# alshai/pfbwt-f

Measured on AMD Instinct MI355X. Metric: Gbases/s end-to-end BWT+SA build; bit-exact .bwt/.sa vs reference, higher is better.
Workload: dtype u8 text / u32 indices / u64 hash; 1 GPU; S-32G; L=32000000, H=1000, seed=1000, w=10, p=100, flags=-r, uint_t=64, n=32000010000, r=83625322, input=text resident in HBM, outputs (.bwt, .ssa, .esa) left in HBM, per_rank=single GPU

## Files before the change

### pfbwt-f_amd/csrc/common.h

```cpp
#pragma once
#include <hip/hip_runtime.h>
#include <cstdint>
#include <cstdio>
#include <cstdlib>
#include <cstring>
#include <chrono>
#include <string>
#include <vector>
#include "../../include/pfbwt_hip.h"
#include "devmem.h"
#include "../../include/pfbwt_hip_dev.h"

namespace pfp {

typedef uint32_t idx_t;

constexpr int BLOCK = 256;
constexpr int WAVE = 64;

constexpr uint8_t Dollar = 2, EndOfWord = 1, EndOfDict = 0;

enum KernelId {
    K_TRIGGER_SCAN, K_PHRASE_ENDS, K_PHRASE_HASH, K_PHRASE_HASH_LONG, K_DEDUP_HEADS, K_DEDUP_LONG,
    K_DICT_BUILD, K_RADIX_HIST, K_RADIX_SCATTER, K_SCAN_REDUCE, K_SCAN_SPINE, K_SCAN_APPLY,
// ... 31 lines not shown
        return base + hi;
    }
    void *reserve_lo(size_t bytes)
    {
        size_t a = (lo + 255) & ~(size_t)255;
        if (a + bytes > hi) { failed = true; want += bytes; return nullptr; }
        lo = a + bytes;
        return base + a;
    }
    bool commit_range(const void *p, size_t bytes) { const size_t o = (size_t)((const char *)p - base); return vm.commit(o, o + bytes); }
    size_t offset_of(const void *p) const { return (size_t)((const char *)p - base); }
    size_t mark_hi() const { return hi; }
    void release_hi(size_t m) { hi = m; }
    size_t mark_lo() const { return lo; }
    void release_lo(size_t m) { lo = m; }
};

struct Tunables {
    int verbose = 0;
    int seg_grid = 768;
    int seg_stage = 1;
    int sort_k = 0;
    int sort_no_table = 0;
    uint32_t class_sort_maxrange = 0;
    int dedup_table_log2 = 0;
    int no_trigger_table = 0;
    uint64_t emit_chunk_rows = 3ULL << 30;
    uint32_t fill_subs = 2;
    uint64_t sample_cap = ~0ULL;
    int no_runaware = 0;
    long big_group_members = -2;
    int force_wide_rows = 0;
    uint64_t ingest_block_bytes = 0;
    int expand_dma = 1;
    int ingest_readers = 0;
    uint32_t emit_group_rows = 4096;
    int dict_text_rounds = -1;
    int force_run_round = 0;
    int int_key_symbols = 3;
    int no_slot_records = 0;
    int group_reduce = 1;
    uint64_t fasta_chunk_bytes = 0;
    int parse_rec = -1;
    int parse_rec_p2 = 4;
    uint64_t parse_rec_min = 1u << 21;
    int parse_rec_depth = 1;
    uint32_t parse_rec_tile_rows = 0;
    int dict_rec = -1;
    int dict_rec_p2 = 16;
    int dedup_variant = -1;
    int64_t dedup_period = 0;
    int64_t dedup_chunk = 0;
    int dedup_packed = 1;
    int dedup_phases = 0;
    int parse_rec_table_log2 = 0;
    uint32_t doc_lds_max = 8192;
};

}

struct pfp_ctx {
    int w = 10; uint64_t p = 100; unsigned flags = 0; int device = 0;
    hipStream_t stream = nullptr;
    pfp::Arena arena;
    size_t arena_request = 0;
    uint64_t err_pos = 0; int err_ch = 0;
    pfp::VmRegion text;
    uint8_t *tb = nullptr; size_t tb_cap = 0; uint64_t n = 0; uint64_t text_hint = 0; uint64_t nseq = 0 ;
    struct RowViewPending { const uint8_t *src = nullptr; uint64_t count = 0, len = 0, stride = 0; } view;
    uint64_t left_ctx = 0;
    uint64_t tb_n = 0;
    int stage = 0;
    uint64_t m = 0, dwords = 0, dsize = 0;
    uint64_t *d_ye = nullptr;
    uint32_t *d_pid = nullptr;
    uint32_t *d_parse = nullptr;
    uint8_t *d_last = nullptr;
    uint8_t *d_dict = nullptr;
    uint32_t *d_ws = nullptr;
    uint32_t *d_wordid = nullptr;
    uint32_t *d_wrank = nullptr;
    uint32_t *d_occ = nullptr;
    uint8_t *d_sdict = nullptr;
    uint32_t *d_gsa = nullptr;
    uint8_t *d_sflag = nullptr;
    uint32_t *d_srank = nullptr;
    uint2 *d_grank = nullptr;
    bool gsa_valid = false;
    uint64_t nrows = 0;
    uint8_t *d_bwlast = nullptr; uint32_t *d_ilist = nullptr; uint64_t *d_bwsai = nullptr;
    uint8_t *d_bwl_il = nullptr;
    uint64_t nout = 0, runs = 0, esa_pairs = 0, easy = 0, hard = 0, slice_begin = 0, slice_rows = 0;
    uint8_t *d_bwt = nullptr; void *d_sa = nullptr; void *d_ssa = nullptr; void *d_esa = nullptr;
    bool have_sa = false, have_rssa = false;
    uint64_t *d_ma = nullptr; uint64_t ma_words = 0;
    size_t ma_lo_mark = (size_t)-1, ma_lo_end = 0;
    void *d_da = nullptr, *d_sda = nullptr, *d_eda = nullptr;
    size_t da_lo_mark = (size_t)-1, da_lo_end = 0;
    size_t lo_after_parse = 0, lo_after_pbwt = 0, emit_scratch_mark = 0;
    bool prof_on = false; uint64_t prof_mask = ~0ULL;
    pfp::ProfRec prof[pfp::K_COUNT_];
    struct PendingEv { hipEvent_t a, b; int id; double bytes; };
    std::vector<PendingEv> pending;
    std::vector<hipEvent_t> ev_pool;
    double stage_ms[3] = {0, 0, 0};
    int hip_err = 0;
    uint8_t *hstage[2] = {nullptr, nullptr}; hipEvent_t hstage_ev[2] = {nullptr, nullptr}; bool hstage_used[2] = {false, false};
    pfp::Tunables tun;
    struct FastaIngest {
        uint8_t *raw[2] = {nullptr, nullptr}; size_t rawcap = 0; bool used[2] = {false, false};
        hipStream_t copy = nullptr; bool copy_ready = false; hipEvent_t ev_copied[2] = {nullptr, nullptr}, ev_free[2] = {nullptr, nullptr};
        uint8_t *tiles = nullptr; size_t tiles_cap = 0;
        unsigned long long *d_tot = nullptr, *h_tot = nullptr;
        uint32_t state = 2; bool started = false; uint64_t records = 0;
        std::vector<uint64_t> rec_raw, rec_pos;
    } fa;
    uint8_t *h_bwt = nullptr; void *h_sa = nullptr;
    uint8_t *ing_buf[16] = {};
    uint64_t ing_next_off = 0;
    std::vector<std::string> doc_names; std::vector<uint64_t> doc_starts;
    uint64_t hash_seed = 0x9E3779B97F4A7C15ULL;
    uint32_t *d_trigtab = nullptr;
};

namespace pfp {

inline hipEvent_t ev_get(pfp_ctx *c)
{
    if (!c->ev_pool.empty()) { hipEvent_t e = c->ev_pool.back(); c->ev_pool.pop_back(); return e; }
    hipEvent_t e; (void)hipEventCreate(&e); return e;
}
inline void prof_collect(pfp_ctx *c)
{
    if (c->pending.empty()) return;
    (void)hipStreamSynchronize(c->stream);
    for (auto &pe : c->pending) {
        float ms = 0; (void)hipEventElapsedTime(&ms, pe.a, pe.b);
        c->prof[pe.id].launches++; c->prof[pe.id].ms += ms; c->prof[pe.id].bytes += pe.bytes;
        c->ev_pool.push_back(pe.a); c->ev_pool.push_back(pe.b);
    }
    c->pending.clear();
}
struct ProfScope {
    pfp_ctx *c; int id; double bytes; hipEvent_t a = nullptr; bool on = false;
    ProfScope(pfp_ctx *c_, int id_, double bytes_) : c(c_), id(id_), bytes(bytes_)
    {
        on = c->prof_on && ((c->prof_mask >> id) & 1ULL);
        if (on) { a = ev_get(c); (void)hipEventRecord(a, c->stream); }
    }
    ~ProfScope()
    {
        if (on) {
            hipEvent_t b = ev_get(c); (void)hipEventRecord(b, c->stream);
            c->pending.push_back({a, b, id, bytes});
            if (c->pending.size() > 4096) prof_collect(c);
        }
    }
};

#define PFP_LAUNCH(ctx, id, bytes, kernel, grid, ...)                                             \
    do {                                                                                          \
        pfp::ProfScope ps_((ctx), (id), (double)(bytes));                                         \
        if ((ctx)->tun.verbose >= 3) { fprintf(stderr, "[pfbwt_hip] launch %s grid %u\n", #kernel, (unsigned)(grid)); fflush(stderr); } \
        hipLaunchKernelGGL(kernel, dim3((unsigned)(grid)), dim3(pfp::BLOCK), 0, (ctx)->stream, __VA_ARGS__); \
        hipError_t le_ = hipGetLastError();             \
        if ((ctx)->tun.verbose >= 3 && le_ == hipSuccess) le_ = hipStreamSynchronize((ctx)->stream);    \
        if (le_ != hipSuccess) { (ctx)->hip_err = (int)le_; (ctx)->err_ch = (int)le_;                 \
            fprintf(stderr, "[pfbwt_hip] launch of %s failed: %s (%s:%d)\n", #kernel, hipGetErrorString(le_), __FILE__, __LINE__); \
            return PFP_E_HIP; }                                                                       \
    } while (0)

#define PFP_LAUNCH_B(ctx, id, bytes, kernel, grid, block, ...)                                    \
    do {                                                                                          \
        pfp::ProfScope ps_((ctx), (id), (double)(bytes));                                         \
// ... 34 lines not shown
```

### pfbwt-f_amd/csrc/parse.h

```cpp
#pragma once
#include "prims.h"

namespace pfp {

typedef uint64_t tpos_t;

__host__ __device__ __forceinline__ uint64_t wang_hash(uint64_t key)
{
    key = (~key) + (key << 21);
    key = key ^ (key >> 24);
    key = (key + (key << 3)) + (key << 8);
    key = key ^ (key >> 14);
    key = (key + (key << 2)) + (key << 4);
    key = key ^ (key >> 28);
    key = key + (key << 31);
    return key;
}

__device__ __forceinline__ uint32_t norm_base(uint32_t c, bool ntoa)
{
    if (c >= 'a' && c <= 'z') c -= 32;
    if (ntoa && !(c == 'A' || c == 'C' || c == 'G' || c == 'T')) c = 'A';
    return c;
}
// ... 15 lines not shown
{
    const uint64_t i = (uint64_t)blockIdx.x * BLOCK + threadIdx.x;
    if (i >= count * (uint64_t)w) return;
    const uint64_t row = i / (uint64_t)w, k = i - row * (uint64_t)w;
    dst[row * pitch + len + k] = 'A';
}

__device__ __forceinline__ uint32_t ntoa_code(uint32_t c)
{
    return (c == 'A' || c == 'N') ? 0u : (c == 'C') ? 1u : (c == 'G') ? 2u : (c == 'T' || c == '-') ? 3u : 5u;
}

__device__ __forceinline__ uint32_t lut8x4(uint32_t hi, uint32_t lo, uint32_t sel)
{
    return __builtin_amdgcn_perm(hi, lo, sel);
}
__device__ __forceinline__ uint32_t pack4(uint32_t x, bool ntoa, uint32_t *bad, uint32_t *out)
{
    const uint32_t h4 = (x >> 1) & 0x07070707u;
    const uint32_t exp4 = lut8x4(0x4E2D0000u, 0x47544341u, h4);
    const uint32_t L = (exp4 & 0x40404040u) >> 1;
    const uint32_t allowed = (x ^ exp4) & ~L;
    uint32_t nz = (((allowed & 0x7F7F7F7Fu) + 0x7F7F7F7Fu) | allowed) & 0x80808080u;
    uint32_t c4 = lut8x4(0x00030000u, 0x02030100u, h4);
    if (ntoa) {
        nz |= (h4 & 0x04040404u) << 5;
        const uint32_t m = (nz >> 7) * 0xFFu;
        *out = (exp4 & ~m) | (0x41414141u & m); c4 &= ~m; *bad = 0;
    } else {
        const uint32_t m = (nz >> 7) * 0xFFu;
        const uint32_t t = x & 0x7F7F7F7Fu;
        const uint32_t lower = (t + 0x1F1F1F1Fu) & ~(t + 0x05050505u) & ~x & 0x80808080u;
        *out = (exp4 & ~m) | ((x ^ (lower >> 2)) & m);
        c4 &= ~m;
        *bad = (((nz >> 7) * 0x01020408u) >> 24) & 0xFu;
    }
    return (c4 * 0x40100401u) >> 24;
}
__device__ __forceinline__ uint32_t pack16(const uint4 &q, bool ntoa, uint32_t *bad , uint4 *normed)
{
    const uint32_t wds[4] = {q.x, q.y, q.z, q.w};
    uint32_t out[4], pk = 0, badm = 0;
#pragma unroll
    for (int i = 0; i < 4; ++i) {
        uint32_t b4;
        pk = (pk << 8) | pack4(wds[i], ntoa, &b4, &out[i]);
        badm |= b4 << (4 * i);
    }
    *bad = badm;
    if (normed) *normed = make_uint4(out[0], out[1], out[2], out[3]);
    return pk;
}

struct DedupText { const uint32_t *Xp; const unsigned long long *Xc; uint64_t nwords; unsigned long long *stats ; };
__device__ __forceinline__ uint32_t codes_lsb_first(uint32_t x)
{
    x = ((x >> 2) & 0x33333333u) | ((x & 0x33333333u) << 2);
    x = ((x >> 4) & 0x0F0F0F0Fu) | ((x & 0x0F0F0F0Fu) << 4);
    return __builtin_bswap32(x);
}
__device__ __forceinline__ bool acgt16(const uint4 &v)
{
    const uint32_t wds[4] = {v.x, v.y, v.z, v.w};
    bool ok = true;
#pragma unroll
    for (int i = 0; i < 4; ++i) {
        const uint32_t h = (wds[i] >> 1) & 0x07070707u;
        ok = ok && wds[i] == lut8x4(0x4E2D0000u, 0x47544341u, h) && !(h & 0x04040404u);
    }
    return ok;
}
__device__ __forceinline__ uint32_t decode4(uint32_t b)
{
    uint32_t s = (b | (b << 12)) & 0x000F000Fu;
    s = (s | (s << 6)) & 0x03030303u;
    return lut8x4(0u, 0x54474341u, s);
}
__device__ __forceinline__ uint64_t decode8(uint32_t x16) { return ((uint64_t)decode4((x16 >> 8) & 0xFFu) << 32) | decode4(x16 & 0xFFu); }

struct DivTest { uint64_t dinv, limit; int k; };
inline DivTest make_divtest(uint64_t p)
{
    DivTest t; t.k = 0;
    uint64_t d = p;
    while (!(d & 1)) { d >>= 1; ++t.k; }
    uint64_t x = d;
    for (int i = 0; i < 5; ++i) x *= 2 - d * x;
    t.dinv = x; t.limit = ~0ULL / p;
    return t;
}
__host__ __device__ __forceinline__ bool divisible(uint64_t h, const DivTest &t)
{
    const uint64_t v = h * t.dinv;
    return (t.k ? ((v >> t.k) | (v << (64 - t.k))) : v) <= t.limit;
}
__global__ __launch_bounds__(BLOCK) void k_trigger_scan(uint8_t *X, uint64_t n, int w, DivTest p, uint64_t kmask, int ntoa,
                                                        uint16_t *mask16, uint64_t *blockcnt, unsigned long long *err_pos)
{
    __shared__ uint32_t pk[BLOCK + 2];
    __shared__ uint32_t red[4];
    const uint64_t t = (uint64_t)blockIdx.x * BLOCK + threadIdx.x;
    const uint64_t base = t * 16;
    uint4 q = make_uint4(0, 0, 0, 0), nq;
    uint32_t bad = 0;
    if (base < n) q = *reinterpret_cast<const uint4 *>(X + base);
    const uint32_t mine = pack16(q, ntoa != 0, &bad, &nq);
    if (base < n) {
        const uint32_t live = (n - base >= 16) ? 0xffffu : ((1u << (unsigned)(n - base)) - 1u);
        if (live != 0xffffu) {
            uint32_t a[4] = {q.x, q.y, q.z, q.w}, b[4] = {nq.x, nq.y, nq.z, nq.w};
            for (int i = 0; i < 16; ++i) if (!((live >> i) & 1)) { b[i >> 2] = (b[i >> 2] & ~(0xffu << (8 * (i & 3)))) | (a[i >> 2] & (0xffu << (8 * (i & 3)))); }
            nq = make_uint4(b[0], b[1], b[2], b[3]);
        }
        *reinterpret_cast<uint4 *>(X + base) = nq;
        bad &= live;
        if (bad) atomicMin(err_pos, (unsigned long long)(base + (uint64_t)(__ffs((int)bad) - 1)));
    }
    pk[threadIdx.x + 2] = mine;
    if (threadIdx.x < 2) {
        const uint64_t first = (uint64_t)blockIdx.x * BLOCK;
        uint32_t hv = 0;
        if (first + threadIdx.x >= 2) {
            uint32_t hb;
            uint4 hq = *reinterpret_cast<const uint4 *>(X + (first + threadIdx.x - 2) * 16);
            hv = pack16(hq, ntoa != 0, &hb, nullptr);
        }
        pk[threadIdx.x] = hv;
    }
    __syncthreads();
    uint64_t kmer = ((uint64_t)pk[threadIdx.x] << 32) | pk[threadIdx.x + 1];
    uint32_t trig = 0;
#pragma unroll
    for (int b = 0; b < 16; ++b) {
        kmer = (kmer << 2) | ((mine >> (30 - 2 * b)) & 3u);
        const uint64_t pos = base + b;
        const uint64_t h = wang_hash(kmer & kmask);
        if (pos < n && pos >= (uint64_t)w && divisible(h, p)) trig |= 1u << b;
    }
    mask16[t] = (uint16_t)trig;
    uint32_t tot;
    (void)block_excl_sum((uint32_t)__popc(trig), red, &tot);
    if (threadIdx.x == 0) blockcnt[blockIdx.x] = tot;
}

constexpr int TS_THREADS = 1024;
constexpr int TS_MAX_W = 10;
constexpr uint32_t TS_TAB_WORDS = 1u << (2 * TS_MAX_W - 5);
__global__ __launch_bounds__(BLOCK) void k_trigger_table(int w, DivTest p, uint32_t *tab)
{
    const uint32_t i = blockIdx.x * BLOCK + threadIdx.x;
    const uint32_t words = (1u << (2 * w)) >= 32u ? (1u << (2 * w)) / 32u : 1u;
    if (i >= words) return;
    uint32_t m = 0;
    for (uint32_t b = 0; b < 32; ++b) { const uint64_t km = (uint64_t)i * 32 + b; if (km < (1ULL << (2 * w)) && divisible(wang_hash(km), p)) m |= 1u << b; }
    tab[i] = m;
}
struct RowView { const uint8_t *src; uint64_t count, len, stride, rowlen ; };
__device__ __forceinline__ uint4 view_load16(const RowView &v, uint64_t r, uint64_t o)
{
    while (o >= v.rowlen) { o -= v.rowlen; ++r; }
    if (r < v.count && o + 16 <= v.len) { uint4 q; __builtin_memcpy(&q, v.src + r * v.stride + o, 16); return q; }
    uint32_t a[4] = {0u, 0u, 0u, 0u};
    for (int k = 0; k < 16; ++k) {
        uint64_t oo = o + (uint64_t)k, rr = r;
        while (oo >= v.rowlen) { oo -= v.rowlen; ++rr; }
        const uint32_t b = rr >= v.count ? 0u : (oo < v.len ? (uint32_t)v.src[rr * v.stride + oo] : (uint32_t)'A');
        a[k >> 2] |= b << (8 * (k & 3));
    }
    return make_uint4(a[0], a[1], a[2], a[3]);
}
template <bool VIEW> __global__ __launch_bounds__(TS_THREADS) void k_trigger_scan_tab(uint8_t *X, uint64_t n, int w, const uint32_t *tab, uint32_t tabwords, uint32_t kmask, int ntoa, uint32_t tiles_per_wg,
                                                                   uint64_t nthreads_total, uint16_t *mask16, uint64_t *blockcnt , unsigned long long *err_pos, RowView rv,
                                                                   uint32_t *Xp , unsigned long long *Xc )
{
    __shared__ uint32_t stab[TS_TAB_WORDS];
    __shared__ uint32_t pk[2][TS_THREADS + 2];
    for (uint32_t i = threadIdx.x; i < tabwords; i += TS_THREADS) stab[i] = tab[i];
    const int lane = threadIdx.x & 63;
    const uint64_t tile0 = (uint64_t)blockIdx.x * tiles_per_wg;
    uint64_t prow = 0, po = 0;
    if (VIEW) { const uint64_t p0 = tile0 * TS_THREADS * 16; prow = p0 / rv.rowlen; po = p0 - prow * rv.rowlen; }
    auto view_tile = [&](uint64_t row, uint64_t o) -> uint4 {
        if (row < rv.count && o + (uint64_t)TS_THREADS * 16 <= rv.len) { uint4 q; __builtin_memcpy(&q, rv.src + row * rv.stride + o + 16u * threadIdx.x, 16); return q; }
        return view_load16(rv, row, o + 16u * threadIdx.x);
    };
    uint32_t requested = 0;
    auto request = [&]() -> uint4 {
        uint4 r = make_uint4(0, 0, 0, 0);
        const uint64_t b = ((tile0 + requested) * TS_THREADS + threadIdx.x) * 16;
        if (requested < tiles_per_wg && b < n) r = VIEW ? view_tile(prow, po) : *reinterpret_cast<const uint4 *>(X + b);
        if (VIEW) { po += (uint64_t)TS_THREADS * 16; while (po >= rv.rowlen) { po -= rv.rowlen; ++prow; } }
        ++requested;
        return r;
    };
    uint4 qa = request(), qb = request(), qc = request();
    for (uint32_t tl = 0; tl < tiles_per_wg; ++tl) {
        const uint64_t first = (tile0 + tl) * TS_THREADS;
        if (first >= nthreads_total) break;
        const uint64_t t = first + threadIdx.x;
        const uint64_t base = t * 16;
        const uint4 q = qa;
        qa = qb; qb = qc; qc = request();
        uint4 nq; uint32_t bad = 0;
        const uint32_t mine = pack16(q, ntoa != 0, &bad, &nq);
        if (base < n) {
            const uint32_t live = (n - base >= 16) ? 0xffffu : ((1u << (unsigned)(n - base)) - 1u);
            if (live != 0xffffu) {
                const uint4 keep = VIEW ? *reinterpret_cast<const uint4 *>(X + base) : q;
                uint32_t a[4] = {keep.x, keep.y, keep.z, keep.w}, b[4] = {nq.x, nq.y, nq.z, nq.w};
                for (int i = 0; i < 16; ++i) if (!((live >> i) & 1)) { b[i >> 2] = (b[i >> 2] & ~(0xffu << (8 * (i & 3)))) | (a[i >> 2] & (0xffu << (8 * (i & 3)))); }
                nq = make_uint4(b[0], b[1], b[2], b[3]);
            }
            if (VIEW || nq.x != q.x || nq.y != q.y || nq.z != q.z || nq.w != q.w) *reinterpret_cast<uint4 *>(X + base) = nq;
            bad &= live;
            if (bad) atomicMin(err_pos, (unsigned long long)(base + (uint64_t)(__ffs((int)bad) - 1)));
        }
        if (Xp) {
            const bool clean = base + 16 <= n && acgt16(nq);
            const unsigned long long cb = __ballot(clean ? 1 : 0);
            if (t < nthreads_total) { Xp[t] = codes_lsb_first(mine); if (lane == 0) Xc[t >> 6] = cb; }
        }
        uint32_t *cur = pk[tl & 1];
        const uint32_t *oth = pk[(tl & 1) ^ 1];
        cur[threadIdx.x + 2] = mine;
        if (threadIdx.x < 2) {
            uint32_t hv = 0;
            if (tl) hv = oth[TS_THREADS + threadIdx.x];
            else if (first + threadIdx.x >= 2) {
                uint32_t hb;
                const uint64_t hp = (first + threadIdx.x - 2) * 16;
                uint4 hq = VIEW ? view_load16(rv, hp / rv.rowlen, hp % rv.rowlen) : *reinterpret_cast<const uint4 *>(X + hp);
                hv = pack16(hq, ntoa != 0, &hb, nullptr);
            }
            cur[threadIdx.x] = hv;
        }
        __syncthreads();
        const uint64_t both = ((uint64_t)cur[threadIdx.x + 1] << 32) | mine;
        const uint32_t amask = (kmask >> 5) << 2, bmask = kmask & 31u;
        const uint8_t *stab8 = reinterpret_cast<const uint8_t *>(stab);
        uint32_t trig = 0;
#pragma unroll
        for (int b = 0; b < 16; ++b) {
            const uint32_t word = *reinterpret_cast<const uint32_t *>(stab8 + ((uint32_t)(both >> (33 - 2 * b)) & amask));
            const uint32_t bit = (uint32_t)(both >> (30 - 2 * b)) & bmask;
            trig |= ((word >> bit) & 1u) << b;
        }
        if (base < (uint64_t)w) trig &= ~((1u << (unsigned)((uint64_t)w - base > 16 ? 16 : (uint64_t)w - base)) - 1u);
        if (base >= n) trig = 0; else if (n - base < 16) trig &= (1u << (unsigned)(n - base)) - 1u;
        if (t < nthreads_total) mask16[t] = (uint16_t)trig;
        uint32_t cnt = (uint32_t)__popc(trig);
#pragma unroll
        for (int d = 32; d >= 1; d >>= 1) cnt += __shfl_xor(cnt, d);
        if (lane == 0 && cnt && t < nthreads_total) atomicAdd(reinterpret_cast<unsigned long long *>(&blockcnt[t / BLOCK]), (unsigned long long)cnt);
    }
}

constexpr int PE_BLOCKS = 8;
__global__ __launch_bounds__(BLOCK) void k_phrase_ends(const uint16_t *mask16, const uint64_t *blockoff, uint64_t ngroups, tpos_t *ye)
{
    __shared__ unsigned long long red[4];
    const uint64_t g0 = (uint64_t)blockIdx.x * PE_BLOCKS;
    uint32_t m[PE_BLOCKS]; unsigned long long c[2] = {0ULL, 0ULL};
#pragma unroll
    for (int b = 0; b < PE_BLOCKS; ++b) {
        m[b] = g0 + b < ngroups ? mask16[(g0 + b) * BLOCK + threadIdx.x] : 0u;
        c[b >> 2] |= (unsigned long long)__popc(m[b]) << (16 * (b & 3));
    }
    unsigned long long tot;
    const unsigned long long e0 = block_excl_sum(c[0], red, &tot), e1 = block_excl_sum(c[1], red, &tot);
#pragma unroll
    for (int b = 0; b < PE_BLOCKS; ++b) {
        if (g0 + b >= ngroups) break;
        uint32_t mm = m[b];
        uint64_t o = blockoff[g0 + b] + (uint32_t)(((b < 4 ? e0 : e1) >> (16 * (b & 3))) & 0xFFFFu);
        const uint64_t t = (g0 + b) * BLOCK + threadIdx.x;
        while (mm) { const int bit = __ffs((int)mm) - 1; mm &= mm - 1; ye[o++] = (tpos_t)(t * 16 + bit + 1); }
    }
}

struct Spans { const tpos_t *ye; const uint32_t *ys32; const uint32_t *ye32; int w; };
__device__ __forceinline__ void phrase_span(const Spans &sp, uint64_t j, tpos_t *ys, uint32_t *len)
{
    if (sp.ys32) { const uint32_t s = sp.ys32[j]; *ys = s; *len = sp.ye32[j] - s + 1u; return; }
    const tpos_t s = j ? sp.ye[j - 1] - (tpos_t)sp.w + 1u : (tpos_t)0;
    *ys = s; *len = (uint32_t)(sp.ye[j] - s + 1u);
}

__device__ __forceinline__ uint64_t ld8(const uint8_t *p) { uint64_t v; __builtin_memcpy(&v, p, 8); return v; }

constexpr uint32_t LONG_PHRASE = 2048;

constexpr uint64_t HT_EMPTY = ~0ULL, HT_NOINFO = ~0ULL;
__device__ __forceinline__ unsigned long long rinfo_make(tpos_t ys, uint32_t len, bool clean) { return ((unsigned long long)ys << 16) | len | ((unsigned long long)clean << 63); }
__device__ __forceinline__ tpos_t rinfo_start(unsigned long long ri) { return (tpos_t)((ri << 1) >> 17); }
constexpr uint32_t HT_MAX_PROBES = 1u << 16;
__host__ __device__ __forceinline__ uint64_t mix64(uint64_t z) { z = (z ^ (z >> 30)) * 0xBF58476D1CE4E5B9ULL; z = (z ^ (z >> 27)) * 0x94D049BB133111EBULL; return z ^ (z >> 31); }
template <typename NEXT> __device__ __forceinline__ uint64_t hash_words(uint32_t len, uint64_t seed, NEXT next )
{
    const uint64_t M = 0xD6E8FEB86659FD93ULL;
    uint64_t h0 = seed ^ ((uint64_t)len * 0x9E3779B97F4A7C15ULL), h1 = h0 ^ 0xA0761D6478BD642FULL, h2 = h0 ^ 0xE7037ED1A0B428DBULL, h3 = h0 ^ 0x8EBC6AF09C88C6E3ULL;
    uint32_t i = 0;
    for (; i + 32 <= len; i += 32) {
        const uint64_t a = next(), b = next(), c = next(), d = next();
        h0 = (h0 ^ a) * M; h1 = (h1 ^ b) * M; h2 = (h2 ^ c) * M; h3 = (h3 ^ d) * M;
        h0 ^= h0 >> 32; h1 ^= h1 >> 32; h2 ^= h2 >> 32; h3 ^= h3 >> 32;
    }
// ... 605 lines not shown
```

### pfbwt-f_amd/csrc/pfbwt_hip.hip

```cpp
#include "common.h"
#include "prims.h"
#include "parse.h"
#include "fasta.h"
#include "sufsort.h"
#include "recsort.h"
#include "dictrec.h"
#include "emit.h"
#include "markers.h"
#include "docarray.h"
#include <map>
#include <sched.h>
#include <thread>
#if defined(__SSE2__)
#include <emmintrin.h>
#endif

using namespace pfp;

#ifndef PFP_BACKEND_NAME
#define PFP_BACKEND_NAME "hip-gfx950"
#endif

static int ensure_arena(pfp_ctx *c, uint64_t n_hint)
{
// ... 8 lines not shown
    }
    want &= ~(size_t)4095;
    if (c->arena.base && c->arena.cap >= want) return PFP_OK;
    VmRegion nv;
    if (nv.reserve(want, c->device) != hipSuccess) { c->arena.want = want; return PFP_E_NOMEM; }
    if (c->arena.base) { PFP_HIP(c, hipStreamSynchronize(c->stream)); (void)hipDeviceSynchronize(); c->arena.vm.destroy(); c->arena.base = nullptr; c->arena.cap = 0; }
    c->arena.vm = nv; nv.base = nullptr;
    c->arena.base = c->arena.vm.base; c->arena.cap = want; c->arena.reset();
    return PFP_OK;
}

static int ensure_text(pfp_ctx *c, uint64_t need_n)
{
    const size_t need = 16 + (((size_t)need_n + 4095) / 4096) * 4096 + 4096 + 64;
    if (c->tb && c->tb_cap >= need) return PFP_OK;
    if (!c->text.live() || need > c->text.va_bytes) {
        size_t fr = 0, tot = 0;
        if (hipMemGetInfo(&fr, &tot) != hipSuccess) { (void)hipGetLastError(); tot = (size_t)1 << 38; }
        size_t va = c->text_hint ? (size_t)c->text_hint + (size_t)c->text_hint / 8 + ((size_t)64 << 20) : (4 * need > ((size_t)64 << 20) ? 4 * need : ((size_t)64 << 20));
        if (!c->text_hint && c->text.live() && va < 2 * c->text.va_bytes) va = 2 * c->text.va_bytes;
        if (!c->text_hint && va > tot && tot > need + need / 4) va = tot;
        if (va < need) va = need + need / 4;
        VmRegion nr;
        if (nr.reserve(va, c->device) != hipSuccess) return PFP_E_NOMEM;
        if (c->tb) {
            if (!nr.commit(0, 16 + (size_t)c->n)) { nr.destroy(); return PFP_E_NOMEM; }
            PFP_HIP(c, hipMemcpyAsync(nr.base, c->tb, 16 + (size_t)c->n, hipMemcpyDeviceToDevice, c->stream));
            PFP_HIP(c, hipStreamSynchronize(c->stream));
            c->text.destroy();
        }
        c->text = nr; nr.base = nullptr;
        c->tb = (uint8_t *)c->text.base; c->tb_cap = 0;
    }
    if (!c->text.commit(0, need)) return PFP_E_NOMEM;
    c->tb_cap = c->text.vmm ? (c->text.lo_edge < c->text.va_bytes ? c->text.lo_edge : c->text.va_bytes) : c->text.va_bytes;
    return PFP_OK;
}

static void reset_results(pfp_ctx *c)
{
    c->stage = 0; c->n = 0; c->nseq = 0; c->tb_n = 0; c->left_ctx = 0; c->view.src = nullptr; c->m = c->dwords = c->dsize = 0; c->nrows = 0; c->nout = c->runs = c->esa_pairs = 0;
    c->gsa_valid = false; c->d_wrank = nullptr; c->d_bwt = nullptr; c->d_sa = c->d_ssa = c->d_esa = nullptr;
    c->d_bwlast = nullptr; c->d_ilist = nullptr; c->d_bwsai = nullptr; c->d_bwl_il = nullptr;
    c->d_ma = nullptr; c->ma_words = 0; c->ma_lo_mark = (size_t)-1;
    c->d_da = c->d_sda = c->d_eda = nullptr; c->da_lo_mark = (size_t)-1;
    c->d_ye = nullptr; c->d_pid = nullptr; c->d_parse = nullptr; c->d_last = nullptr; c->d_dict = nullptr; c->d_ws = nullptr; c->d_wordid = nullptr;
    c->d_occ = nullptr; c->d_sdict = nullptr; c->d_gsa = nullptr; c->d_grank = nullptr; c->d_srank = nullptr; c->d_sflag = nullptr;
    c->arena.reset();
    c->fa.started = false; c->fa.state = 2; c->fa.records = 0; c->fa.rec_raw.clear(); c->fa.rec_pos.clear();
}

static const char *const tunable_names[] = {"verbose", "seg_grid", "seg_stage", "sort_k", "sort_no_table", "class_sort_maxrange", "dedup_table_log2", "no_trigger_table",
                                            "emit_chunk_rows", "fill_subs", "sample_cap", "no_runaware", "big_group_members", "force_wide_rows", "fasta_chunk_bytes", "ingest_block_bytes", "emit_group_rows", "no_slot_records", "dict_text_rounds", "int_key_symbols", "force_run_round",
                                            "ingest_readers", "expand_dma", "parse_rec", "parse_rec_p2", "parse_rec_min", "parse_rec_depth", "parse_rec_tile_rows", "parse_rec_table_log2", "dict_rec", "dict_rec_p2", "dedup_variant", "dedup_phases", "dedup_period", "dedup_chunk", "doc_lds_max", "dedup_packed", "group_reduce"};
static int set_tunable(pfp_ctx *c, const char *key, long long v)
{
    Tunables &t = c->tun;
    if (!strcmp(key, "verbose")) t.verbose = (int)v;
    else if (!strcmp(key, "seg_grid")) t.seg_grid = (int)v;
    else if (!strcmp(key, "seg_stage")) t.seg_stage = (int)v;
    else if (!strcmp(key, "sort_k")) t.sort_k = (int)v;
    else if (!strcmp(key, "sort_no_table")) t.sort_no_table = (int)v;
    else if (!strcmp(key, "class_sort_maxrange")) t.class_sort_maxrange = (uint32_t)v;
    else if (!strcmp(key, "dedup_table_log2")) t.dedup_table_log2 = (int)v;
    else if (!strcmp(key, "no_trigger_table")) t.no_trigger_table = (int)v;
    else if (!strcmp(key, "emit_chunk_rows")) t.emit_chunk_rows = v > 0 ? (uint64_t)v : (3ULL << 30);
    else if (!strcmp(key, "fill_subs")) t.fill_subs = (uint32_t)v;
    else if (!strcmp(key, "sample_cap")) t.sample_cap = v < 0 ? ~0ULL : (uint64_t)v;
    else if (!strcmp(key, "no_runaware")) t.no_runaware = (int)v;
    else if (!strcmp(key, "big_group_members")) t.big_group_members = (long)v;
    else if (!strcmp(key, "force_wide_rows")) t.force_wide_rows = (int)v;
    else if (!strcmp(key, "fasta_chunk_bytes")) t.fasta_chunk_bytes = v > 0 ? (uint64_t)v : 0;
    else if (!strcmp(key, "ingest_block_bytes")) t.ingest_block_bytes = v > 0 ? (uint64_t)v : 0;
    else if (!strcmp(key, "emit_group_rows")) t.emit_group_rows = v > 0 ? (uint32_t)v : 0u;
    else if (!strcmp(key, "no_slot_records")) t.no_slot_records = (int)v;
    else if (!strcmp(key, "dict_text_rounds")) t.dict_text_rounds = (int)v;
    else if (!strcmp(key, "int_key_symbols")) t.int_key_symbols = (int)v;
    else if (!strcmp(key, "force_run_round")) t.force_run_round = (int)v;
    else if (!strcmp(key, "ingest_readers")) t.ingest_readers = (int)v;
    else if (!strcmp(key, "expand_dma")) t.expand_dma = (int)v;
    else if (!strcmp(key, "parse_rec")) t.parse_rec = (int)v;
    else if (!strcmp(key, "parse_rec_p2")) t.parse_rec_p2 = (int)v;
    else if (!strcmp(key, "parse_rec_min")) t.parse_rec_min = v > 0 ? (uint64_t)v : 0;
    else if (!strcmp(key, "parse_rec_depth")) t.parse_rec_depth = (int)v;
    else if (!strcmp(key, "parse_rec_tile_rows")) t.parse_rec_tile_rows = v > 0 ? (uint32_t)v : 0u;
    else if (!strcmp(key, "parse_rec_table_log2")) t.parse_rec_table_log2 = (int)v;
    else if (!strcmp(key, "dict_rec")) t.dict_rec = (int)v;
    else if (!strcmp(key, "dict_rec_p2")) t.dict_rec_p2 = (int)v;
    else if (!strcmp(key, "dedup_variant")) t.dedup_variant = (int)v;
    else if (!strcmp(key, "dedup_phases")) t.dedup_phases = (int)v;
    else if (!strcmp(key, "dedup_packed")) t.dedup_packed = (int)v;
    else if (!strcmp(key, "group_reduce")) t.group_reduce = (int)v;
    else if (!strcmp(key, "dedup_period")) t.dedup_period = (int64_t)v;
    else if (!strcmp(key, "dedup_chunk")) t.dedup_chunk = (int64_t)v;
    else if (!strcmp(key, "doc_lds_max")) t.doc_lds_max = v < 2 ? 2u : v > (long long)DOC_LDS_CAP ? DOC_LDS_CAP : (uint32_t)v;
    else return PFP_E_ARG;
    return PFP_OK;
}
static void load_tunables_from_env(pfp_ctx *c)
{
    if (getenv("PFP_VERBOSE")) c->tun.verbose = 1;
    const char *hooks = getenv("PFP_TEST_HOOKS");
    if (!hooks || strcmp(hooks, "1")) return;
    for (const char *name : tunable_names) {
        char env[64] = "PFP_"; size_t k = 4;
        for (const char *q = name; *q && k + 1 < sizeof env; ++q) env[k++] = (char)((*q >= 'a' && *q <= 'z') ? *q - 32 : *q);
        env[k] = 0;
        const char *e = getenv(env);
        if (e) (void)set_tunable(c, name, *e ? atoll(e) : 1LL);
    }
}

extern "C" {

const char *pfp_backend(void) { return PFP_BACKEND_NAME; }
int pfp_debug_set(pfp_ctx *c, const char *key, long long value) { return (c && key) ? set_tunable(c, key, value) : PFP_E_ARG; }

const char *pfp_strerror(int s)
{
    switch (s) {
    case PFP_OK: return "ok";
    case PFP_E_ARG: return "invalid argument";
    case PFP_E_INVALID_CHAR: return "error, invalid character";
    case PFP_E_TOO_LARGE: return "input too long for 32-bit device indices";
    case PFP_E_NOMEM: return "device workspace exhausted";
    case PFP_E_HIP: return "HIP runtime error";
    case PFP_E_ONE_WORD: return "error: only one dict word total. Re-run with a smaller p modulus";
    case PFP_E_STATE: return "call order violated";
    case PFP_E_CORRUPT: return "something went wrong!";
    case PFP_E_IO: return "failed to open file!";
    default: return "unknown status";
    }
}

pfp_ctx *pfp_create(int w, uint64_t p, unsigned flags, int device, uint64_t workspace_bytes, int *status)
{
    int st = PFP_OK;
    pfp_ctx *c = nullptr;
    if (w < 1 || w > 32 || p == 0) st = PFP_E_ARG;
    else {
        int ndev = 0;
        if (hipGetDeviceCount(&ndev) != hipSuccess || ndev <= 0 || device < 0 || device >= ndev) st = PFP_E_HIP;
        else if (hipSetDevice(device) != hipSuccess) st = PFP_E_HIP;
        else {
            c = new pfp_ctx();
// ... 703 lines not shown
};

static int parse_finalize_impl(pfp_ctx *c, pfp_parse_sizes *out, bool shard_only);
static int parse_finalize_entry(pfp_ctx *c, pfp_parse_sizes *out, bool shard_only)
{
    if (!c) return PFP_E_ARG;
    if (c->stage != 0) return PFP_E_STATE;
    if (c->n == 0) return PFP_E_ARG;
    PFP_HIP(c, hipSetDevice(c->device));
    ArenaGuard g(c);
    const int rc = g.done(parse_finalize_impl(c, out, shard_only));
    if (rc != PFP_OK) { c->m = c->dwords = c->dsize = 0; c->gsa_valid = false; }
    return rc;
}
int pfp_parse_finalize(pfp_ctx *c, pfp_parse_sizes *out) { return parse_finalize_entry(c, out, false); }
int pfp_parse_finalize_shard(pfp_ctx *c, pfp_parse_sizes *out) { return parse_finalize_entry(c, out, true); }
static int parse_finalize_impl(pfp_ctx *c, pfp_parse_sizes *out, bool shard_only)
{
    HostTimer timer;
    const uint64_t n = c->n; const int w = c->w;
    PFP_TRY(ensure_arena(c, n));
    c->arena.reset();
    uint8_t *X = c->tb + 16; const uint8_t *Y = c->tb + 15;
    PFP_HIP(c, hipMemsetAsync(c->tb, Dollar, 16, c->stream));
    PFP_HIP(c, hipMemsetAsync(X + n, Dollar, (size_t)w, c->stream));
    const size_t mk = c->arena.mark_hi();

    const unsigned gts = nblocks(n, 16 * BLOCK);
    uint16_t *mask16; uint64_t *blockcnt; uint32_t *d_u32; unsigned long long *d_err;
    PFP_ALLOC_HI(c, mask16, uint16_t, (size_t)gts * BLOCK);
    PFP_ALLOC_HI(c, blockcnt, uint64_t, (size_t)gts + 1);
    PFP_ALLOC_HI(c, d_u32, uint32_t, 8);
    PFP_ALLOC_HI(c, d_err, unsigned long long, 1);
    PFP_HIP(c, hipMemsetAsync(d_err, 0xff, 8, c->stream));
    PFP_HIP(c, hipMemsetAsync(d_u32, 0, 32, c->stream));
    const uint64_t kmask = (w == 32) ? 0ULL : ((1ULL << (2 * w)) - 1ULL);
    const bool no_trigtab = c->tun.no_trigger_table != 0;
    DedupText dt = {nullptr, nullptr, 0, nullptr};
    if (w <= TS_MAX_W && !no_trigtab && c->tun.dedup_packed) {
        const uint64_t nw = (uint64_t)gts * BLOCK;
        uint32_t *xp; unsigned long long *xc;
        PFP_ALLOC_HI(c, xp, uint32_t, nw + 128);
        PFP_ALLOC_HI(c, xc, unsigned long long, nw / 64 + 1);
        dt.Xp = xp + 64; dt.Xc = xc; dt.nwords = nw;
    }
    if (c->view.src && !(w <= TS_MAX_W && !no_trigtab)) PFP_TRY(flush_view(c));
    if (w <= TS_MAX_W && !no_trigtab) {
        const uint32_t tabwords = (1u << (2 * w)) >= 32u ? (1u << (2 * w)) / 32u : 1u;
        if (!c->d_trigtab) {
            PFP_HIP(c, hipMalloc((void **)&c->d_trigtab, (size_t)TS_TAB_WORDS * 4));
            PFP_LAUNCH(c, K_MISC, tabwords * 4, k_trigger_table, nblocks(tabwords, BLOCK), w, make_divtest(c->p), c->d_trigtab);
        }
        const uint64_t nthreads_total = (uint64_t)gts * BLOCK;
        const uint64_t tiles = (nthreads_total + TS_THREADS - 1) / TS_THREADS;
        uint32_t tpw = (uint32_t)(tiles / 1024); if (tpw < 1) tpw = 1; if (tpw > 64) tpw = 64;
        PFP_HIP(c, hipMemsetAsync(blockcnt, 0, ((size_t)gts + 1) * 8, c->stream));
        if (c->view.src) {
            const RowView rv = {c->view.src, c->view.count, c->view.len, c->view.stride, c->view.len + (uint64_t)w};
            PFP_LAUNCH_B(c, K_TRIGGER_SCAN, 2 * n + n / 8, (k_trigger_scan_tab<true>), (tiles + tpw - 1) / tpw, TS_THREADS, X, n, w, (const uint32_t *)c->d_trigtab, tabwords, (uint32_t)kmask,
                         (int)((c->flags & PFP_FLAG_NON_ACGT_TO_A) != 0), tpw, nthreads_total, mask16, blockcnt, d_err, rv, (uint32_t *)dt.Xp, (unsigned long long *)dt.Xc);
            c->view.src = nullptr;
        } else
        PFP_LAUNCH_B(c, K_TRIGGER_SCAN, n + n / 8, (k_trigger_scan_tab<false>), (tiles + tpw - 1) / tpw, TS_THREADS, X, n, w, (const uint32_t *)c->d_trigtab, tabwords, (uint32_t)kmask,
                     (int)((c->flags & PFP_FLAG_NON_ACGT_TO_A) != 0), tpw, nthreads_total, mask16, blockcnt, d_err, RowView{nullptr, 0, 0, 0, 1}, (uint32_t *)dt.Xp, (unsigned long long *)dt.Xc);
    } else
    PFP_LAUNCH(c, K_TRIGGER_SCAN, n * 2 + n / 8, k_trigger_scan, gts, X, n, w, make_divtest(c->p), kmask, (int)((c->flags & PFP_FLAG_NON_ACGT_TO_A) != 0), mask16, blockcnt, d_err);
    PFP_TRY((device_scan<uint64_t, 0>(c, blockcnt, blockcnt, gts, blockcnt + gts)));
    uint64_t ntrig = 0; unsigned long long herr = 0;
    PFP_HIP(c, hipMemcpyAsync(&herr, d_err, 8, hipMemcpyDeviceToHost, c->stream));
    PFP_HIP(c, hipMemcpyAsync(&ntrig, blockcnt + gts, 8, hipMemcpyDeviceToHost, c->stream));
    PFP_HIP(c, hipStreamSynchronize(c->stream));
    if (herr != ~0ULL) {
        uint8_t ch = 0;
        PFP_HIP(c, hipMemcpy(&ch, X + herr, 1, hipMemcpyDeviceToHost));
        c->err_pos = herr; c->err_ch = ch;
        return PFP_E_INVALID_CHAR;
    }
    const uint64_t m = ntrig + 1;
    if (m > 0xFFFFFFFEULL - 64) return PFP_E_TOO_LARGE;
    c->m = m;
    PFP_ALLOC_LO(c, c->d_ye, tpos_t, m);
    PFP_LAUNCH(c, K_PHRASE_ENDS, n / 8 + m * 4, k_phrase_ends, nblocks(gts, PE_BLOCKS), (const uint16_t *)mask16, (const uint64_t *)blockcnt, (uint64_t)gts, c->d_ye);
    PFP_LAUNCH(c, K_MISC, 8, k_set_u64, 1, c->d_ye, m - 1, (uint64_t)(n + (uint64_t)w));

    Spans sp; sp.ye = c->d_ye; sp.ys32 = nullptr; sp.ye32 = nullptr; sp.w = w;
    uint64_t dwords = 0; uint32_t *rep, *occw;
    PFP_ALLOC_LO(c, c->d_pid, uint32_t, m);
    PFP_ALLOC_LO(c, c->d_last, uint8_t, m);
    PFP_TRY(dedup_strings(c, Y, sp, m, n + (uint64_t)w + 1 + m * (uint64_t)w, c->d_pid, &dwords, &rep, &occw, c->d_last, dt));
    PFP_TRY(build_dictionary(c, Y, sp, rep, dwords));
    if (!shard_only) PFP_TRY(finish_parse(c, occw));
    PFP_HIP(c, hipStreamSynchronize(c->stream));
    c->arena.release_hi(mk);
    c->stage = 1;
    c->lo_after_parse = c->arena.mark_lo();
    c->stage_ms[0] = timer.ms();
    if (out) { out->n = n; out->m = m; out->dwords = c->dwords; out->dsize = c->dsize; }
    return PFP_OK;
}

__global__ __launch_bounds__(BLOCK) void k_merge_spans(const uint32_t *ws, uint32_t dwords, uint32_t ubase, uint32_t coff, uint32_t frag0, uint32_t frag0_ys, uint32_t frag0_ye,
                                                       uint32_t fragl, uint32_t fragl_ys, uint32_t fragl_ye, uint32_t *ys, uint32_t *ye)
{
    const uint32_t k = blockIdx.x * BLOCK + threadIdx.x;
    if (k >= dwords) return;
    uint32_t a = ubase + ws[k], b = ubase + ws[k + 1] - 2u;
    if (k == frag0) { a = frag0_ys; b = frag0_ye; }
    if (k == fragl) { a = fragl_ys; b = fragl_ye; }
    ys[coff + k] = a; ye[coff + k] = b;
}
__global__ __launch_bounds__(BLOCK) void k_merge_phrases(const uint32_t *pid, const tpos_t *ye, const uint8_t *last, uint32_t m, uint32_t j0, uint32_t goff, uint32_t coff, tpos_t shift,
                                                         const uint32_t *cand_id, tpos_t junction_ye, uint32_t junction_last, int has_junction,
                                                         uint32_t *gpid, tpos_t *gye, uint8_t *glast, uint32_t *occw)
{
    const uint32_t j = j0 + blockIdx.x * BLOCK + threadIdx.x;
    if (j >= m) return;
    const uint32_t g = goff + j - j0;
// ... 1525 lines not shown
```

Baseline: 130.3 Gbases/s.

## Restructure trigger scan into per-wave contiguous runs with DPP neighbor exchange

The trigger-scan kernel now gives each wave a contiguous run of 64-thread chunks, where before whole 1024-thread tiles were synchronised with __syncthreads and exchanged neighbour words through LDS. Each lane gets its predecessor's packed word via DPP and the previous chunk's last lane via readlane. Per-block counts come from a ballot-based wave reduction written directly, which removes the atomics and the memset. It also adds a fast validation/packing path that falls back to the slow pack only when a wave sees invalid chars, and sizes the grid from the CU count. In exchange, each wave's chunks are processed serially, which may reduce memory-level parallelism, and the code is more complex.

```diff
diff --git a/pfbwt-f_amd/csrc/common.h b/pfbwt-f_amd/csrc/common.h
--- a/pfbwt-f_amd/csrc/common.h
+++ b/pfbwt-f_amd/csrc/common.h
@@ -107,6 +107,7 @@
     int64_t dedup_period = 0;
     int64_t dedup_chunk = 0;
     int dedup_packed = 1;
+    int scan_waves = 16;
     int dedup_phases = 0;
     int parse_rec_table_log2 = 0;
     uint32_t doc_lds_max = 8192;
@@ -175,6 +176,7 @@
     uint64_t ing_next_off = 0;
     std::vector<std::string> doc_names; std::vector<uint64_t> doc_starts;
     uint64_t hash_seed = 0x9E3779B97F4A7C15ULL;
+    int num_cus = 0;
     uint32_t *d_trigtab = nullptr;
 };
 
diff --git a/pfbwt-f_amd/csrc/parse.h b/pfbwt-f_amd/csrc/parse.h
--- a/pfbwt-f_amd/csrc/parse.h
+++ b/pfbwt-f_amd/csrc/parse.h
@@ -91,6 +91,29 @@
     return pk;
 }
 
+__device__ __forceinline__ uint32_t pack16_valid(const uint4 &q, bool ntoa, uint32_t *inv, uint32_t *dashn, uint4 *normed)
+{
+    const uint32_t wds[4] = {q.x, q.y, q.z, q.w};
+    uint32_t out[4], pk = 0, nzs = 0, hs = 0;
+#pragma unroll
+    for (int i = 0; i < 4; ++i) {
+        const uint32_t x = wds[i];
+        const uint32_t h4 = (x >> 1) & 0x07070707u;
+        const uint32_t exp4 = lut8x4(0x4E2D0000u, 0x47544341u, h4);
+        const uint32_t L = (exp4 & 0x40404040u) >> 1;
+        const uint32_t allowed = (x ^ exp4) & ~L;
+        nzs |= ((allowed & 0x7F7F7F7Fu) + 0x7F7F7F7Fu) | allowed;
+        hs |= h4;
+        const uint32_t c4 = lut8x4(0x00030000u, 0x02030100u, h4);
+        out[i] = exp4;
+        pk = (pk << 8) | ((c4 * 0x40100401u) >> 24);
+    }
+    *dashn = hs & 0x04040404u;
+    *inv = (nzs & 0x80808080u) | (ntoa ? *dashn : 0u);
+    *normed = make_uint4(out[0], out[1], out[2], out[3]);
+    return pk;
+}
+
 struct DedupText { const uint32_t *Xp; const unsigned long long *Xc; uint64_t nwords; unsigned long long *stats ; };
 __device__ __forceinline__ uint32_t codes_lsb_first(uint32_t x)
 {
@@ -183,6 +206,9 @@
 }
 
 constexpr int TS_THREADS = 1024;
+constexpr uint32_t TS_WAVES = TS_THREADS / 64;
+constexpr uint32_t TS_CHUNKS = BLOCK / 64;
+constexpr uint32_t TS_WG_PER_CU = 4;
 constexpr int TS_MAX_W = 10;
 constexpr uint32_t TS_TAB_WORDS = 1u << (2 * TS_MAX_W - 5);
 __global__ __launch_bounds__(BLOCK) void k_trigger_table(int w, DivTest p, uint32_t *tab)
@@ -191,7 +217,7 @@
     const uint32_t words = (1u << (2 * w)) >= 32u ? (1u << (2 * w)) / 32u : 1u;
     if (i >= words) return;
     uint32_t m = 0;
-    for (uint32_t b = 0; b < 32; ++b) { const uint64_t km = (uint64_t)i * 32 + b; if (km < (1ULL << (2 * w)) && divisible(wang_hash(km), p)) m |= 1u << b; }
+    for (uint32_t b = 0; b < 32; ++b) { const uint64_t km = ((uint64_t)i * 32 + b) & ((1ULL << (2 * w)) - 1ULL); if (divisible(wang_hash(km), p)) m |= 1u << b; }
     tab[i] = m;
 }
 struct RowView { const uint8_t *src; uint64_t count, len, stride, rowlen ; };
@@ -208,40 +234,81 @@
     }
     return make_uint4(a[0], a[1], a[2], a[3]);
 }
-template <bool VIEW> __global__ __launch_bounds__(TS_THREADS) void k_trigger_scan_tab(uint8_t *X, uint64_t n, int w, const uint32_t *tab, uint32_t tabwords, uint32_t kmask, int ntoa, uint32_t tiles_per_wg,
-                                                                   uint64_t nthreads_total, uint16_t *mask16, uint64_t *blockcnt , unsigned long long *err_pos, RowView rv,
-                                                                   uint32_t *Xp , unsigned long long *Xc )
+__device__ __forceinline__ uint32_t lane_pred(uint32_t v, uint32_t first)
+{
+#if !defined(PFBWT_EMU_HIP_RUNTIME_H)
+    return (uint32_t)__builtin_amdgcn_update_dpp((int)first, (int)v, 0x138 , 0xf, 0xf, false);
+#else
+    const uint32_t u = __shfl_up(v, 1u);
+    return (threadIdx.x & 63) ? u : first;
+#endif
+}
+__device__ __forceinline__ uint32_t lane_last(uint32_t v)
+{
+#if !defined(PFBWT_EMU_HIP_RUNTIME_H)
+    return (uint32_t)__builtin_amdgcn_readlane((int)v, 63);
+#else
+    return __shfl(v, 63);
+#endif
+}
+__device__ __forceinline__ uint32_t wave_number()
+{
+#if !defined(PFBWT_EMU_HIP_RUNTIME_H)
+    return (uint32_t)__builtin_amdgcn_readfirstlane((int)(threadIdx.x >> 6));
+#else
+    return threadIdx.x >> 6;
+#endif
+}
+template <bool VIEW> __global__ __launch_bounds__(TS_THREADS) void k_trigger_scan_tab(uint8_t *X, uint64_t n, int w, const uint32_t *tab, uint32_t tabwords, uint32_t kmask, int ntoa, uint32_t groups_per_wg,
+                                                                   uint32_t waves , uint32_t run , uint64_t nthreads_total, uint16_t *mask16, uint64_t *blockcnt ,
+                                                                   unsigned long long *err_pos, RowView rv, uint32_t *Xp , unsigned long long *Xc )
 {
     __shared__ uint32_t stab[TS_TAB_WORDS];
-    __shared__ uint32_t pk[2][TS_THREADS + 2];
     for (uint32_t i = threadIdx.x; i < tabwords; i += TS_THREADS) stab[i] = tab[i];
-    const int lane = threadIdx.x & 63;
-    const uint64_t tile0 = (uint64_t)blockIdx.x * tiles_per_wg;
+    __syncthreads();
+    const uint32_t lane = threadIdx.x & 63, wv = wave_number();
+    if (wv >= waves) return;
+    const uint64_t g0 = (uint64_t)blockIdx.x * groups_per_wg;
+    const uint64_t gall = nthreads_total / BLOCK, gend = g0 + groups_per_wg < gall ? g0 + groups_per_wg : gall;
+    const uint64_t c0 = (g0 + (uint64_t)wv * run) * TS_CHUNKS;
+    const uint64_t cend = c0 + (uint64_t)run * TS_CHUNKS < gend * TS_CHUNKS ? c0 + (uint64_t)run * TS_CHUNKS : gend * TS_CHUNKS;
+    uint64_t rc = c0;
     uint64_t prow = 0, po = 0;
-    if (VIEW) { const uint64_t p0 = tile0 * TS_THREADS * 16; prow = p0 / rv.rowlen; po = p0 - prow * rv.rowlen; }
-    auto view_tile = [&](uint64_t row, uint64_t o) -> uint4 {
-        if (row < rv.count && o + (uint64_t)TS_THREADS * 16 <= rv.len) { uint4 q; __builtin_memcpy(&q, rv.src + row * rv.stride + o + 16u * threadIdx.x, 16); return q; }
-        return view_load16(rv, row, o + 16u * threadIdx.x);
-    };
-    uint32_t requested = 0;
+    if (VIEW) { const uint64_t p0 = rc * 1024u; prow = p0 / rv.rowlen; po = p0 - prow * rv.rowlen; }
+    uint4 hq = make_uint4(0, 0, 0, 0);
     auto request = [&]() -> uint4 {
         uint4 r = make_uint4(0, 0, 0, 0);
-        const uint64_t b = ((tile0 + requested) * TS_THREADS + threadIdx.x) * 16;
-        if (requested < tiles_per_wg && b < n) r = VIEW ? view_tile(prow, po) : *reinterpret_cast<const uint4 *>(X + b);
-        if (VIEW) { po += (uint64_t)TS_THREADS * 16; while (po >= rv.rowlen) { po -= rv.rowlen; ++prow; } }
-        ++requested;
+        const uint64_t b0 = rc * 1024u;
+        if (rc < cend && b0 < n) {
+            if (rc == c0 && rc && lane == 0) {
+                if (VIEW) hq = po >= 16 ? view_load16(rv, prow, po - 16) : view_load16(rv, (b0 - 16) / rv.rowlen, (b0 - 16) % rv.rowlen);
+                else hq = *reinterpret_cast<const uint4 *>(X + b0 - 16);
+            }
+            const uint64_t b = b0 + 16u * lane;
+            if (VIEW) {
+                if (prow < rv.count && po + 1024u <= rv.len) __builtin_memcpy(&r, rv.src + prow * rv.stride + po + 16u * lane, 16);
+                else if (b < n) r = view_load16(rv, prow, po + 16u * lane);
+            } else if (b < n) r = *reinterpret_cast<const uint4 *>(X + b);
+        }
+        ++rc;
+        if (VIEW) {
+            po += 1024u;
+            if (po >= rv.rowlen) { if (po - rv.rowlen < rv.rowlen) { po -= rv.rowlen; ++prow; } else { const uint64_t k = po / rv.rowlen; prow += k; po -= k * rv.rowlen; } }
+        }
         return r;
     };
     uint4 qa = request(), qb = request(), qc = request();
-    for (uint32_t tl = 0; tl < tiles_per_wg; ++tl) {
-        const uint64_t first = (tile0 + tl) * TS_THREADS;
-        if (first >= nthreads_total) break;
-        const uint64_t t = first + threadIdx.x;
-        const uint64_t base = t * 16;
+    uint32_t carry = 0, cnt = 0;
+    for (uint64_t pc = c0; pc < cend; ++pc) {
+        const bool head = pc == c0;
         const uint4 q = qa;
         qa = qb; qb = qc; qc = request();
-        uint4 nq; uint32_t bad = 0;
-        const uint32_t mine = pack16(q, ntoa != 0, &bad, &nq);
+        const uint64_t t = pc * 64u + lane;
+        const uint64_t base = t * 16;
+        uint4 nq; uint32_t bad = 0, inv, dashn;
+        uint32_t mine = pack16_valid(q, ntoa != 0, &inv, &dashn, &nq);
+        bool acgt = dashn == 0;
+        if (__any(inv != 0)) { mine = pack16(q, ntoa != 0, &bad, &nq); acgt = acgt16(nq); }
         if (base < n) {
             const uint32_t live = (n - base >= 16) ? 0xffffu : ((1u << (unsigned)(n - base)) - 1u);
             if (live != 0xffffu) {
@@ -255,42 +322,34 @@
             if (bad) atomicMin(err_pos, (unsigned long long)(base + (uint64_t)(__ffs((int)bad) - 1)));
         }
         if (Xp) {
-            const bool clean = base + 16 <= n && acgt16(nq);
+            const bool clean = base + 16 <= n && acgt;
             const unsigned long long cb = __ballot(clean ? 1 : 0);
-            if (t < nthreads_total) { Xp[t] = codes_lsb_first(mine); if (lane == 0) Xc[t >> 6] = cb; }
-        }
-        uint32_t *cur = pk[tl & 1];
-        const uint32_t *oth = pk[(tl & 1) ^ 1];
-        cur[threadIdx.x + 2] = mine;
-        if (threadIdx.x < 2) {
-            uint32_t hv = 0;
-            if (tl) hv = oth[TS_THREADS + threadIdx.x];
-            else if (first + threadIdx.x >= 2) {
-                uint32_t hb;
-                const uint64_t hp = (first + threadIdx.x - 2) * 16;
-                uint4 hq = VIEW ? view_load16(rv, hp / rv.rowlen, hp % rv.rowlen) : *reinterpret_cast<const uint4 *>(X + hp);
-                hv = pack16(hq, ntoa != 0, &hb, nullptr);
-            }
-            cur[threadIdx.x] = hv;
-        }
-        __syncthreads();
-        const uint64_t both = ((uint64_t)cur[threadIdx.x + 1] << 32) | mine;
-        const uint32_t amask = (kmask >> 5) << 2, bmask = kmask & 31u;
+            Xp[t] = codes_lsb_first(mine); if (lane == 0) Xc[pc] = cb;
+        }
+        uint32_t first = carry;
+        if (head) { uint32_t hb; first = pc ? pack16(hq, ntoa != 0, &hb, nullptr) : 0u; }
+        const uint32_t prev = lane_pred(mine, first);
+        carry = lane_last(mine);
+        const uint64_t both = ((uint64_t)prev << 32) | mine;
+        const uint32_t amask = (kmask >> 5) << 2;
         const uint8_t *stab8 = reinterpret_cast<const uint8_t *>(stab);
+        uint32_t word[16];
+#pragma unroll
+        for (int b = 15; b >= 0; --b) word[b] = *reinterpret_cast<const uint32_t *>(stab8 + ((uint32_t)(both >> (33 - 2 * b)) & amask));
         uint32_t trig = 0;
 #pragma unroll
-        for (int b = 0; b < 16; ++b) {
-            const uint32_t word = *reinterpret_cast<const uint32_t *>(stab8 + ((uint32_t)(both >> (33 - 2 * b)) & amask));
-            const uint32_t bit = (uint32_t)(both >> (30 - 2 * b)) & bmask;
-            trig |= ((word >> bit) & 1u) << b;
-        }
+        for (int b = 15; b >= 0; --b) trig = (trig << 1) | ((word[b] >> ((uint32_t)(both >> (30 - 2 * b)) & 31u)) & 1u);
         if (base < (uint64_t)w) trig &= ~((1u << (unsigned)((uint64_t)w - base > 16 ? 16 : (uint64_t)w - base)) - 1u);
         if (base >= n) trig = 0; else if (n - base < 16) trig &= (1u << (unsigned)(n - base)) - 1u;
-        if (t < nthreads_total) mask16[t] = (uint16_t)trig;
-        uint32_t cnt = (uint32_t)__popc(trig);
-#pragma unroll
-        for (int d = 32; d >= 1; d >>= 1) cnt += __shfl_xor(cnt, d);
-        if (lane == 0 && cnt && t < nthreads_total) atomicAdd(reinterpret_cast<unsigned long long *>(&blockcnt[t / BLOCK]), (unsigned long long)cnt);
+        mask16[t] = (uint16_t)trig;
+        cnt += (uint32_t)__popc(trig);
+        if ((pc & (TS_CHUNKS - 1)) == TS_CHUNKS - 1) {
+            uint32_t tot = 0;
+#pragma unroll
+            for (int b = 0; b < 7; ++b) tot += (uint32_t)__popcll(__ballot((int)((cnt >> b) & 1u))) << b;
+            if (lane == 0) blockcnt[pc / TS_CHUNKS] = tot;
+            cnt = 0;
+        }
     }
 }
 
diff --git a/pfbwt-f_amd/csrc/pfbwt_hip.hip b/pfbwt-f_amd/csrc/pfbwt_hip.hip
--- a/pfbwt-f_amd/csrc/pfbwt_hip.hip
+++ b/pfbwt-f_amd/csrc/pfbwt_hip.hip
@@ -84,7 +84,7 @@
 
 static const char *const tunable_names[] = {"verbose", "seg_grid", "seg_stage", "sort_k", "sort_no_table", "class_sort_maxrange", "dedup_table_log2", "no_trigger_table",
                                             "emit_chunk_rows", "fill_subs", "sample_cap", "no_runaware", "big_group_members", "force_wide_rows", "fasta_chunk_bytes", "ingest_block_bytes", "emit_group_rows", "no_slot_records", "dict_text_rounds", "int_key_symbols", "force_run_round",
-                                            "ingest_readers", "expand_dma", "parse_rec", "parse_rec_p2", "parse_rec_min", "parse_rec_depth", "parse_rec_tile_rows", "parse_rec_table_log2", "dict_rec", "dict_rec_p2", "dedup_variant", "dedup_phases", "dedup_period", "dedup_chunk", "doc_lds_max", "dedup_packed", "group_reduce"};
+                                            "ingest_readers", "expand_dma", "parse_rec", "parse_rec_p2", "parse_rec_min", "parse_rec_depth", "parse_rec_tile_rows", "parse_rec_table_log2", "dict_rec", "dict_rec_p2", "dedup_variant", "dedup_phases", "dedup_period", "dedup_chunk", "doc_lds_max", "dedup_packed", "group_reduce", "scan_waves"};
 static int set_tunable(pfp_ctx *c, const char *key, long long v)
 {
     Tunables &t = c->tun;
@@ -123,6 +123,7 @@
     else if (!strcmp(key, "dedup_phases")) t.dedup_phases = (int)v;
     else if (!strcmp(key, "dedup_packed")) t.dedup_packed = (int)v;
     else if (!strcmp(key, "group_reduce")) t.group_reduce = (int)v;
+    else if (!strcmp(key, "scan_waves")) t.scan_waves = (int)v;
     else if (!strcmp(key, "dedup_period")) t.dedup_period = (int64_t)v;
     else if (!strcmp(key, "dedup_chunk")) t.dedup_chunk = (int64_t)v;
     else if (!strcmp(key, "doc_lds_max")) t.doc_lds_max = v < 2 ? 2u : v > (long long)DOC_LDS_CAP ? DOC_LDS_CAP : (uint32_t)v;
@@ -932,17 +933,29 @@
             PFP_LAUNCH(c, K_MISC, tabwords * 4, k_trigger_table, nblocks(tabwords, BLOCK), w, make_divtest(c->p), c->d_trigtab);
         }
         const uint64_t nthreads_total = (uint64_t)gts * BLOCK;
-        const uint64_t tiles = (nthreads_total + TS_THREADS - 1) / TS_THREADS;
-        uint32_t tpw = (uint32_t)(tiles / 1024); if (tpw < 1) tpw = 1; if (tpw > 64) tpw = 64;
-        PFP_HIP(c, hipMemsetAsync(blockcnt, 0, ((size_t)gts + 1) * 8, c->stream));
+        if (!c->num_cus) {
+#if !defined(PFBWT_EMU_HIP_RUNTIME_H)
+            int cus = 0;
+            PFP_HIP(c, hipDeviceGetAttribute(&cus, hipDeviceAttributeMultiprocessorCount, c->device));
+            c->num_cus = cus > 0 ? cus : 1;
+#else
+            c->num_cus = 2;
+#endif
+        }
+        uint64_t nwg = ((uint64_t)gts + 3) / 4;
+        if (nwg > (uint64_t)c->num_cus * TS_WG_PER_CU) nwg = (uint64_t)c->num_cus * TS_WG_PER_CU;
+        const uint32_t gpw = (uint32_t)((gts + nwg - 1) / nwg);
+        nwg = (gts + (uint64_t)gpw - 1) / gpw;
+        const uint32_t waves = c->tun.scan_waves < 1 ? 1u : c->tun.scan_waves > (int)TS_WAVES ? TS_WAVES : (uint32_t)c->tun.scan_waves;
+        const uint32_t run = (gpw + waves - 1) / waves;
         if (c->view.src) {
             const RowView rv = {c->view.src, c->view.count, c->view.len, c->view.stride, c->view.len + (uint64_t)w};
-            PFP_LAUNCH_B(c, K_TRIGGER_SCAN, 2 * n + n / 8, (k_trigger_scan_tab<true>), (tiles + tpw - 1) / tpw, TS_THREADS, X, n, w, (const uint32_t *)c->d_trigtab, tabwords, (uint32_t)kmask,
-                         (int)((c->flags & PFP_FLAG_NON_ACGT_TO_A) != 0), tpw, nthreads_total, mask16, blockcnt, d_err, rv, (uint32_t *)dt.Xp, (unsigned long long *)dt.Xc);
+            PFP_LAUNCH_B(c, K_TRIGGER_SCAN, 2 * n + n / 8, (k_trigger_scan_tab<true>), nwg, TS_THREADS, X, n, w, (const uint32_t *)c->d_trigtab, tabwords, (uint32_t)kmask,
+                         (int)((c->flags & PFP_FLAG_NON_ACGT_TO_A) != 0), gpw, waves, run, nthreads_total, mask16, blockcnt, d_err, rv, (uint32_t *)dt.Xp, (unsigned long long *)dt.Xc);
             c->view.src = nullptr;
         } else
-        PFP_LAUNCH_B(c, K_TRIGGER_SCAN, n + n / 8, (k_trigger_scan_tab<false>), (tiles + tpw - 1) / tpw, TS_THREADS, X, n, w, (const uint32_t *)c->d_trigtab, tabwords, (uint32_t)kmask,
-                     (int)((c->flags & PFP_FLAG_NON_ACGT_TO_A) != 0), tpw, nthreads_total, mask16, blockcnt, d_err, RowView{nullptr, 0, 0, 0, 1}, (uint32_t *)dt.Xp, (unsigned long long *)dt.Xc);
+        PFP_LAUNCH_B(c, K_TRIGGER_SCAN, n + n / 8, (k_trigger_scan_tab<false>), nwg, TS_THREADS, X, n, w, (const uint32_t *)c->d_trigtab, tabwords, (uint32_t)kmask,
+                     (int)((c->flags & PFP_FLAG_NON_ACGT_TO_A) != 0), gpw, waves, run, nthreads_total, mask16, blockcnt, d_err, RowView{nullptr, 0, 0, 0, 1}, (uint32_t *)dt.Xp, (unsigned long long *)dt.Xc);
     } else
     PFP_LAUNCH(c, K_TRIGGER_SCAN, n * 2 + n / 8, k_trigger_scan, gts, X, n, w, make_divtest(c->p), kmask, (int)((c->flags & PFP_FLAG_NON_ACGT_TO_A) != 0), mask16, blockcnt, d_err);
     PFP_TRY((device_scan<uint64_t, 0>(c, blockcnt, blockcnt, gts, blockcnt + gts)));
```

Result: faster. 134.0 Gbases/s (median of 6 runs) (+2.8%).
